# CUHK-AIM-Group/Depth-Aware-Endoscopy-SR

Measured on AMD Instinct MI355X. Metric: LR frames/sec fwd+bwd at x8 (128x160 LR), higher is better.
Workload: dtype f32; 1 GPU; Kvasir x8 synthetic, batch=16 per GPU, fp32, DepthNet nb=16 nf=64 L=256 K=10 (BASELINE.json configs[1]); step = fwd + L1 + dynamic loss + bwd + Adam; global_batch=16, scale=8, parallelism=dp1, mode=train, device=cuda, full=False, hip_graph=False

## Files before the change

### depth-aware-endoscopy-sr_amd/csrc/conv_split_bf16.hip

```cpp
#include "bf16.h"
#include "conv_kernels.h"

typedef _Float16 f16_t;
typedef _Float16 f16x8 __attribute__((ext_vector_type(8)));
typedef _Float16 f16x2_t __attribute__((ext_vector_type(2)));

#define SP_HW 34
#define SP_NWV 8
#define SP_NTHR 512
#define SP_TH 16
#define SP_HPIX (18 * SP_HW)
#define SP_NHP 5
#define SP_HBYTES (SP_NHP * SP_NTHR * 16)
#define SP_EPITCH 144

DASR_DEVICE_CONST __attribute__((aligned(64))) unsigned sp_zero_page[64] = {0};

struct ConvSplitArgs {
    const float* x;
    const bf16_t* ws;
    const float* bias;
    const float* residual;
    float* y;
    int B, H, W, Cin, Cout, accumulate, act, ps_r;
    int tiles_x, tiles_y, nsl, nitems, Q, G8;
    const float* xmax;
    const float* wmax;
    float* ymax;
    const float* xact;
    int fact, fps;
};

template <int N>
__device__ __forceinline__ void sp_wait_vm() {
#ifndef DASR_HIPEMU
    asm volatile("s_waitcnt vmcnt(%0)" ::"n"(N) : "memory");
#endif
}

__device__ __forceinline__ void sp_wait_vm_n(int n) {
    switch (n) {
#define SP_W(N) case N: sp_wait_vm<N>(); break;
        SP_W(0) SP_W(1) SP_W(2) SP_W(3) SP_W(4) SP_W(5) SP_W(6) SP_W(7) SP_W(8) SP_W(9) SP_W(10) SP_W(11) SP_W(12)
#undef SP_W
        default: sp_wait_vm<0>(); break;
    }
}

__device__ __forceinline__ void sp_split3(const float (&x)[8], bf16x8& a0, bf16x8& a1, bf16x8& a2) {
#pragma unroll
    for (int e = 0; e < 8; e += 2) {
        const bf16x2_t h0 = dasr_f2bf2(x[e], x[e + 1]);
        const float r0 = x[e] - dasr_bf2f(h0[0]), r1 = x[e + 1] - dasr_bf2f(h0[1]);
        const bf16x2_t h1 = dasr_f2bf2(r0, r1);
        const float s0 = r0 - dasr_bf2f(h1[0]), s1 = r1 - dasr_bf2f(h1[1]);
        const bf16x2_t h2 = dasr_f2bf2(s0, s1);
        a0[e] = h0[0]; a0[e + 1] = h0[1];
        a1[e] = h1[0]; a1[e + 1] = h1[1];
        a2[e] = h2[0]; a2[e + 1] = h2[1];
    }
}

__host__ __device__ static inline int sp_scale_exp(float m) {
// ... 271 lines not shown
                for (int j = 0; j < 2; ++j) {
                    const int v = lane + 64 * u, cq = v & 7, px = 2 * (v >> 3) + j;
                    const float4 s = *(const float4*)(scr + px * SP_EPITCH + 16 * cq);
                    float o[4] = {s.x, s.y, s.z, s.w};
                    if (NP == 2) {
                        const float* bp = sBias + n0 + 4 * cq;
#pragma unroll
                        for (int t = 0; t < 4; ++t) o[t] = fmaf(o[t], inv, bp[t]);
                    }
                    const float xv[4] = {xa[m][u][j].x, xa[m][u][j].y, xa[m][u][j].z, xa[m][u][j].w};
#pragma unroll
                    for (int t = 0; t < 4; ++t) r[m][u][j][t] = o[t] * (xv[t] > 0.f ? 1.f : dneg);
                }
            DASR_WAVE_SYNC();
        }
        if (rowok) {
            const size_t Cq = (size_t)4 * a.Cout;
#pragma unroll
            for (int u = 0; u < 2; ++u) {
                const int v = lane + 64 * u, cq = v & 7, P = v >> 3;
                if (2 * P >= wvalid) continue;
                float* yp = a.y + (((size_t)bb * (a.H >> 1) + (gy0 >> 1)) * (a.W >> 1) + (x0 >> 1) + P) * Cq + 4 * (n0 + 4 * cq);
#pragma unroll
                for (int t = 0; t < 4; ++t) {
                    const float4 q = make_float4(r[0][u][0][t], r[0][u][1][t], r[1][u][0][t], r[1][u][1][t]);
                    *(float4*)(yp + 4 * t) = q;
                    om = dasr_amax4(om, q);
                }
            }
        }
    }
}

template <int NT, int NP, int RW = 2, int CW = 1>
__global__ void __launch_bounds__(64 * (SP_TH / RW), RW == 4 ? 1 : 2) k_conv3x3_split(ConvSplitArgs a) {
    DASR_DYN_SMEM(smem);
    typedef SpFrag<NP> F;
    static_assert(CW == 1 || (CW == 2 && NP == 2 && RW == 2 && (NT % 2) == 0), "channel halves: fp16 x 2, eight waves");
    constexpr int MR = RW * CW, NW = NT / CW;
    constexpr int NWV = SP_TH / RW, NTHR = 64 * NWV, NHP = SP_HBYTES / (16 * NTHR);
    constexpr int NTILE = 32 * NT, PIECE = NTILE * 32, SLAB = NP * PIECE;
    constexpr int WP = SLAB / 16;
    constexpr int WQ = WP / NTHR, WR = (WP - WQ * NTHR) / 64;
    char* const sH = smem;
    constexpr int TPS = NP == 2 ? 3 : 1, NS = 9 / TPS;
    constexpr int R = 3, D = 2;
    char* const sW = smem + 2 * SP_HBYTES;
    float* const sBias = (float*)(sW + R * TPS * SLAB);
    float* const sRed = sBias + a.Cout;
    const int tid = threadIdx.x, lane = tid & 63, wv = DASR_UNIFORM((int)(tid >> 6));
    const int li = lane & 31, lh = lane >> 5;
    const int wr = wv / CW, wc = wv % CW;
    const int nwq = WQ + (wv < WR ? 1 : 0);
    const dasr_lds_addr_t ldsH = DASR_LDS_ADDR(sH) + 1024 * wv, ldsW = DASR_LDS_ADDR(sW) + 1024 * wv;

    const int xcd = blockIdx.x & 7, jwg = blockIdx.x >> 3;
    const int ibeg = xcd * a.Q;
    const int iend = ibeg + a.Q < a.nitems ? ibeg + a.Q : a.nitems;
    int item = ibeg + jwg;
    if (item >= iend) {
        if (a.ymax) dasr_amax_commit_idle(a.ymax, dasr_flat_wg(), dasr_flat_nwg());
        return;
    }
    const int NC = a.Cin >> 4;
    const int pixb = a.Cin * 4, rowb = a.W * pixb;
    const size_t sampb = (size_t)a.H * rowb;
    const char* const zp = (const char*)sp_zero_page;

    for (int i = tid; i < a.Cout; i += NTHR) sBias[i] = a.bias ? a.bias[i] : 0.f;
    sp_scales_gather<NP>(a.xmax, a.wmax, sRed);
    __syncthreads();
    const SpScale sc = sp_scales_take<NP>(sRed);

    int x0, y0, n0, bb;
    auto decode = [&](int it, int& ox0, int& oy0, int& on0, int& ob) {
        const int ns = it % a.nsl, pt = it / a.nsl;
        const int tile = pt % (a.tiles_x * a.tiles_y);
        ob = pt / (a.tiles_x * a.tiles_y);
        ox0 = (tile % a.tiles_x) * 32;
        oy0 = (tile / a.tiles_x) * SP_TH;
        on0 = ns * NTILE;
    };
    decode(item, x0, y0, n0, bb);
    int hoff[NHP];
    unsigned hok = 0;
    const char* hxb;
    auto halo_setup = [&](int fx0, int fy0, int fb, bool real) {
        hxb = (const char*)a.x + (size_t)fb * sampb;
        const int org = (fy0 - 1) * rowb + (fx0 - 1) * pixb;
        int t = tid;
#ifndef DASR_HIPEMU
        asm volatile("" : "+v"(t));
#endif
        hok = 0;
#pragma unroll
        for (int u = 0; u < NHP; ++u) {
            const int P = (t >> 2) + (NTHR / 4) * u;
            const int pr = P / SP_HW, pc = P - pr * SP_HW;
            hoff[u] = org + pr * rowb + pc * pixb + 16 * ((t & 3) ^ ((P >> 2) & 3));
            const bool ok = real && P < SP_HPIX && (unsigned)(fy0 - 1 + pr) < (unsigned)a.H && (unsigned)(fx0 - 1 + pc) < (unsigned)a.W;
            hok |= ok ? (1u << u) : 0u;
        }
    };
    auto halo_issue = [&](int u, int cc, int buf) {
        const char* src = ((hok >> u) & 1u) ? hxb + hoff[u] + 64 * cc : zp;
// ... 108 lines not shown
                typename F::type A[RW][NP];
#pragma unroll
                for (int m = 0; m < RW; ++m) {
                    const int P = Pq + (m + dy) * SP_HW + dx;
                    const int key = (P >> 2) & 3;
                    if constexpr (NP == 2) {
                        A[m][0] = sp_frag(hb + P * 64, lh, key, 0);
                        A[m][1] = sp_frag(hb + P * 64, lh, key, 1);
                    } else {
                        const float4 lo = *(const float4*)(hb + P * 64 + (((2 * lh) ^ key) << 4));
                        const float4 hi = *(const float4*)(hb + P * 64 + (((2 * lh + 1) ^ key) << 4));
                        const float xv[8] = {lo.x, lo.y, lo.z, lo.w, hi.x, hi.y, hi.z, hi.w};
                        F::split(xv, sc.sx, A[m]);
                    }
                }
                DASR_SETPRIO(1);
#pragma unroll
                for (int n = 0; n < NT; ++n) {
                    typename F::type Bw[NP];
#pragma unroll
                    for (int j = 0; j < NP; ++j) Bw[j] = *(const typename F::type*)(wb + j * PIECE + n * 1024);
#pragma unroll
                    for (int m = 0; m < RW; ++m) acc[m][n] = F::mma(Bw, A[m], acc[m][n]);
                }
                DASR_SETPRIO(0);
                }
                }
            }
            par ^= 1;
        }

        DASR_RAW_BARRIER();
        char* const scr = sH + (par ^ 1) * SP_HBYTES + wv * (32 * SP_EPITCH);
        sp_epilogue<NW, NP, MR>(acc, a, scr, sBias, sc.inv, x0, y0, n0 + 32 * NW * wc, bb, MR * wr, lane, li, lh, om);
        if (!has_next) break;
        item = nitem; x0 = nx0; y0 = ny0; n0 = nn0; bb = nb;
    }
    sp_wait_vm<0>();
    if (a.ymax) dasr_amax_commit(a.ymax, om, sRed, dasr_flat_wg(), dasr_flat_nwg());
}

template <int NP, int NT = 1, bool FUSE = false>
__global__ void __launch_bounds__(SP_NTHR, 2) k_conv3x3_split_n32(ConvSplitArgs a) {
    DASR_DYN_SMEM(smem);
    typedef SpFrag<NP> F;
    constexpr int NTILE = 32 * NT, PIECE = NTILE * 32, SLAB = NP * PIECE;
    constexpr int WCH = 9 * SLAB, WPC = WCH / 16;
    constexpr int WPT = SLAB / 16;
    constexpr int WU = (WPC + SP_NTHR - 1) / SP_NTHR, WLAST = (WPC - (WU - 1) * SP_NTHR) / 64;
    char* const sH = smem;
    char* const sW = smem + 2 * SP_HBYTES;
    float* const sBias = (float*)(sW + 2 * WCH);
    float* const sRed = sBias + a.Cout;
    const int tid = threadIdx.x, lane = tid & 63, wv = DASR_UNIFORM((int)(tid >> 6));
    const int li = lane & 31, lh = lane >> 5;
    const dasr_lds_addr_t ldsH = DASR_LDS_ADDR(sH) + 1024 * wv, ldsW = DASR_LDS_ADDR(sW) + 1024 * wv;

    const int xcd = blockIdx.x & 7, jwg = blockIdx.x >> 3;
    const int ibeg = xcd * a.Q;
    const int iend = ibeg + a.Q < a.nitems ? ibeg + a.Q : a.nitems;
    int item = ibeg + jwg;
    if (item >= iend) {
        if (a.ymax) dasr_amax_commit_idle(a.ymax, dasr_flat_wg(), dasr_flat_nwg());
        return;
    }
    const int NC = a.Cin >> 4;
    const int pixb = a.Cin * 4, rowb = a.W * pixb;
    const size_t sampb = (size_t)a.H * rowb;
    const char* const zp = (const char*)sp_zero_page;

    for (int i = tid; i < a.Cout; i += SP_NTHR) sBias[i] = a.bias ? a.bias[i] : 0.f;
// ... 296 lines not shown
extern "C" int dasr_conv3x3_split2_weights_slabs(int Cin, int Cout) {
    if (Cin <= 0 || Cout <= 0 || (Cin % 32) != 0 || (Cout % 32) != 0) return 0;
    return (int)sp_weight_slabs_all(Cin, Cout);
}
extern "C" int dasr_conv3x3_split2_weights_multi(const dasr_split_job* jobs_host, const dasr_split_job* jobs_device, int njobs,
                                                 void* stream) {
    DASR_CHECK_PTR(jobs_host); DASR_CHECK_PTR(jobs_device);
    DASR_CHECK_SHAPE(njobs > 0);
    long long total = 0;
    for (int j = 0; j < njobs; ++j) {
        const dasr_split_job& J = jobs_host[j];
        DASR_CHECK_PTR(J.w_packed); DASR_CHECK_PTR(J.w_split); DASR_CHECK_PTR(J.wmax);
        DASR_CHECK_SHAPE(J.Cin > 0 && J.Cout > 0 && (J.Cin % 32) == 0 && (J.Cout % 32) == 0);
        DASR_CHECK_SHAPE(J.wg_begin == total);
        total += sp_weight_slabs_all(J.Cin, J.Cout);
        DASR_CHECK_SHAPE(total < (1ll << 30));
    }
    DASR_LAUNCH(k_split_weights_multi, dim3((unsigned)total), dim3(256), 0, stream, jobs_device, njobs);
    DASR_RETURN_LAUNCH_STATUS();
}
template <int NP>
static int sp_launch(ConvSplitArgs& a, void* stream) {
    const int NT = sp_ntile(a.Cout) / 32;
    a.tiles_x = (a.W + 31) / 32;
    a.tiles_y = (a.H + SP_TH - 1) / SP_TH;
    a.nsl = a.Cout / (32 * NT);
    a.nitems = a.tiles_x * a.tiles_y * a.B * a.nsl;
    a.Q = (a.nitems + 7) / 8;
    a.G8 = a.Q < 32 ? a.Q : 32;
    if ((dasr_get_conv_bf16_impl() & 3) == 2) a.G8 = 1;
    const bool chunk2 = NT == 2 && NP == 2 && (dasr_get_conv_bf16_impl() & 512) != 0;
    const size_t lds = 2 * (size_t)SP_HBYTES +
                       (NT == 1 || chunk2 ? 2 * (size_t)(9 * NP * 32 * NT * 32) : 3 * (size_t)((NP == 2 ? 3 : 1) * NP * 32 * NT * 32)) +
                       sizeof(float) * (size_t)(a.Cout + 32);
    if (lds > 160 * 1024) return DASR_E_UNSUPPORTED;
    const dim3 grid(8 * a.G8);
    if (a.xact) {
        if (NT != 1 || NP != 2) return DASR_E_UNSUPPORTED;
        DASR_LAUNCH((k_conv3x3_split_n32<2, 1, true>), grid, dim3(SP_NTHR), lds, stream, a);
    }
    else if (NT == 4 && NP == 2 && (dasr_get_conv_bf16_impl() & 256) != 0)
        DASR_LAUNCH((k_conv3x3_split<4, 2, 4>), grid, dim3(256), lds, stream, a);
    else if (NT == 4 && NP == 2 && (dasr_get_conv_bf16_impl() & 1024) == 0)
        DASR_LAUNCH((k_conv3x3_split<4, 2, 2, 2>), grid, dim3(SP_NTHR), lds, stream, a);
    else if (NT == 2 && NP == 2 && (dasr_get_conv_bf16_impl() & 1024) != 0)
        DASR_LAUNCH((k_conv3x3_split<2, 2, 2, 2>), grid, dim3(SP_NTHR), lds, stream, a);
    else if (NT == 4) DASR_LAUNCH((k_conv3x3_split<4, NP>), grid, dim3(SP_NTHR), lds, stream, a);
    else if (chunk2)  DASR_LAUNCH((k_conv3x3_split_n32<2, 2>), grid, dim3(SP_NTHR), lds, stream, a);
    else if (NT == 2) DASR_LAUNCH((k_conv3x3_split<2, NP>), grid, dim3(SP_NTHR), lds, stream, a);
    else              DASR_LAUNCH((k_conv3x3_split_n32<NP>), grid, dim3(SP_NTHR), lds, stream, a);
    DASR_RETURN_LAUNCH_STATUS();
}
static int sp_fwd(const float* x, const float* xmax, const unsigned short* w_split, const float* wmax, const float* bias,
                  const float* residual, float* y, float* ymax, int B, int H, int W, int Cin, int Cout, int act, int ps_r,
                  void* stream) {
    DASR_CHECK_PTR(x); DASR_CHECK_PTR(w_split); DASR_CHECK_PTR(y);
    DASR_CHECK_SHAPE(B > 0);
    if (!dasr_conv3x3_split_supported(H, W, Cin, Cout)) return DASR_E_UNSUPPORTED;
    if (act < 0 || act > 2) return DASR_E_UNSUPPORTED;
    if (ps_r < 1) ps_r = 1;
    if (ps_r > 2 || (ps_r == 2 && (residual != nullptr || (Cout % 128) != 0))) return DASR_E_UNSUPPORTED;
    ConvSplitArgs a{x, (const bf16_t*)w_split, bias, residual, y, B, H, W, Cin, Cout, 0, act, ps_r, 0, 0, 0, 0, 0, 0, xmax, wmax, ymax};
    return xmax ? sp_launch<2>(a, stream) : sp_launch<3>(a, stream);
}
extern "C" int dasr_conv3x3_fwd_split(const float* x, const unsigned short* w_split, const float* bias,
                                      const float* residual, float* y, int B, int H, int W, int Cin, int Cout, int act,
                                      int ps_r, void* stream) {
    return sp_fwd(x, nullptr, w_split, nullptr, bias, residual, y, nullptr, B, H, W, Cin, Cout, act, ps_r, stream);
}
// ... 9 lines not shown
    DASR_CHECK_SHAPE(B > 0);
    if (!dasr_conv3x3_split_supported(H, W, Cin, Cout)) return DASR_E_UNSUPPORTED;
    const size_t mode1 = (size_t)9 * (dmax ? 2 : 3) * Cin * Cout;
    ConvSplitArgs a{dconv, (const bf16_t*)w_split + mode1, nullptr, nullptr, dx, B, H, W, Cout, Cin,
                    accumulate, DASR_ACT_NONE, 1, 0, 0, 0, 0, 0, 0, dmax, wmax, nullptr};
    return dmax ? sp_launch<2>(a, stream) : sp_launch<3>(a, stream);
}
extern "C" int dasr_conv3x3_dgrad_split(const float* dconv, const unsigned short* w_split, float* dx, int accumulate, int B,
                                        int H, int W, int Cin, int Cout, void* stream) {
    return sp_dgrad(dconv, nullptr, w_split, nullptr, dx, accumulate, B, H, W, Cin, Cout, stream);
}
extern "C" int dasr_conv3x3_dgrad_split2(const float* dconv, const float* dmax, const unsigned short* w_split, const float* wmax,
                                         float* dx, int accumulate, int B, int H, int W, int Cin, int Cout, void* stream) {
    DASR_CHECK_PTR(dmax); DASR_CHECK_PTR(wmax);
    return sp_dgrad(dconv, dmax, w_split, wmax, dx, accumulate, B, H, W, Cin, Cout, stream);
}
extern "C" int dasr_conv3x3_dgrad_act_supported(int H, int W, int Cin, int Cout, int act, int ps_r, int accumulate) {
    if (Cin != 32 || !dasr_conv3x3_split_supported(H, W, Cin, Cout)) return 0;
    if (act != DASR_ACT_NONE && act != DASR_ACT_RELU && act != DASR_ACT_LRELU02) return 0;
    if (ps_r == 1) return 1;
    return (ps_r == 2 && (H % 2) == 0 && (W % 2) == 0 && !accumulate) ? 1 : 0;
}
extern "C" int dasr_conv3x3_dgrad_act_split2(const float* dconv, const float* dmax, const unsigned short* w_split, const float* wmax,
                                             const float* x_act, float* dprev, float* dprev_amax, int accumulate, int B, int H,
                                             int W, int Cin, int Cout, int act, int ps_r, void* stream) {
    DASR_CHECK_PTR(dconv); DASR_CHECK_PTR(dmax); DASR_CHECK_PTR(w_split); DASR_CHECK_PTR(wmax); DASR_CHECK_PTR(x_act);
    DASR_CHECK_PTR(dprev);
    DASR_CHECK_SHAPE(B > 0);
    if (!dasr_conv3x3_dgrad_act_supported(H, W, Cin, Cout, act, ps_r, accumulate)) return DASR_E_UNSUPPORTED;
    const size_t mode1 = (size_t)9 * 2 * Cin * Cout;
    ConvSplitArgs a{dconv, (const bf16_t*)w_split + mode1, nullptr, nullptr, dprev, B, H, W, Cout, Cin,
                    accumulate ? 1 : 0, DASR_ACT_NONE, 1, 0, 0, 0, 0, 0, 0, dmax, wmax, dprev_amax, x_act, act, ps_r};
    return sp_launch<2>(a, stream);
}

#define SW_TW 32
__host__ __device__ constexpr int sw_th(int MT, int NTW) { return MT * NTW == 4 ? 2 : (MT * NTW == 2 ? 4 : 8); }

struct SplitWgradArgs {
    const float* xmax;
    const float* dmax;
    const float* x;
    const float* dy;
    float* slabs;
    float* bslabs;
    int B, H, W, Cin, Cout;
    int P, ntiles;
};

__device__ __forceinline__ void sp_split_pair(float v0, float v1, bf16x2_t& h0, bf16x2_t& h1, bf16x2_t& h2) {
    h0 = dasr_f2bf2(v0, v1);
    const float r0 = v0 - dasr_bf2f(h0[0]), r1 = v1 - dasr_bf2f(h0[1]);
    h1 = dasr_f2bf2(r0, r1);
    h2 = dasr_f2bf2(r0 - dasr_bf2f(h1[0]), r1 - dasr_bf2f(h1[1]));
}

__device__ __forceinline__ void sp_split_pair2(float v0, float v1, float s, f16x2_t& h0, f16x2_t& h1) {
    v0 *= s; v1 *= s;
    h0[0] = (f16_t)v0; h0[1] = (f16_t)v1;
    h1[0] = (f16_t)(v0 - (float)h0[0]); h1[1] = (f16_t)(v1 - (float)h0[1]);
}

template <int MT, int NTW, int NP>
__global__ void __launch_bounds__(256, 2) k_conv3x3_wgrad_split(SplitWgradArgs a) {
    DASR_DYN_SMEM(smem);
    typedef SpFrag<NP> F;
// ... 459 lines not shown
```

### depth-aware-endoscopy-sr_amd/graph.py

```python
import math

import torch

from . import ops
from .tape import Tape, Var, accum


FUSE_DGRAD_ACT = False
FUSE_C9_DGRAD_ACT = True
FUSE_SPLIT_DGRAD_ACT = True

SIDE_STREAM = True
import os as _os
import threading as _threading
TAIL_WGRAD_SIDE = False
FUSE_INSTNORM_STATS = False
ENCODER_S2D = True
SPLIT_BF16 = True
SPLIT_WGRAD = True
SPLIT_PIECES = 2
FUSE_AMAX = True
SPLIT_CONV9 = True
SPLIT_MIN_PIXELS = 1 << 14
WGRAD_STREAM = False
_SIDE = {}
_SIDE_LOCK = _threading.Lock()


def _side_stream(device, which="branch"):
    key = (str(device), which)
    with _SIDE_LOCK:
        if key not in _SIDE:
            _SIDE[key] = torch.cuda.Stream(device=device, priority=-1)
        return _SIDE[key]


def _folded(tape, key, tensors, make):
    cache = tape.fold_cache
    if tape.enabled or cache is None or key is None:
        return make()
    ver = tuple((t.data_ptr(), ops.tensor_version(t)) for t in tensors)
    key = key + (str(tensors[0].device),)
    hit = cache.get(key)
# ... 248 lines not shown
            y = ops.conv3x3_fwd_split(x.data, w.split, bias.data if bias is not None else None, w.data.shape[4],
                                      residual.data if residual is not None else None, act, ps_r)
    elif (SPLIT_BF16 and SPLIT_PIECES == 2 and SPLIT_CONV9 and f32 and w.data.dtype == torch.float32 and stride == 1 and pad == 4
          and not transposed and tuple(w.data.shape[1:3]) == (9, 9) and act == ops.ACT_NONE and ps_r == 1 and residual is None
          and x.data.shape[0] * x.data.shape[1] * x.data.shape[2] >= SPLIT_MIN_PIXELS
          and ops.conv9_split_supported(x.data.shape[1], x.data.shape[2], w.data.shape[3], w.data.shape[4])):
        if w.split is None:
            w.split = ("c9", _folded(tape, ("c9max", "@%x" % w.data.data_ptr()), [w.data], lambda: ops.absmax(w.data[0])))
            if w.pack is not None:
                tape.prepack.note_split(w.pack, w.split)
        y = ops.conv9_fwd_split2(x.data, _amax(x), w.data, w.split[1], bias.data if bias is not None else None)
    else:
        am = want_amax(tape, x.data) if (f32 and x.data.shape[3] in (1, 3) and ps_r == 1) else None
        y = ops.conv2d_fwd(x.data, w.data, bias.data if bias is not None else None,
                           residual.data if residual is not None else None, stride, pad, transposed, act, ps_r, out_dtype,
                           amax=am)
    needs = x.requires_grad or w.requires_grad or (bias is not None and bias.requires_grad) or \
        (residual is not None and residual.requires_grad)
    out = Var(y, needs)
    out.stats = stats
    x.uses += 1
    if residual is not None:
        residual.uses += 1
    if (act != ops.ACT_NONE or ps_r > 1) and residual is None:
        out.epilogue = (act, ps_r)
        out.epilogue_split = isinstance(w.split, tuple)
    if act != ops.ACT_NONE or ps_r > 1:
        out.act_rec = (act, ps_r)
        out.epilogue_split = isinstance(w.split, tuple)
    KH, KW, Cin, Cout = w.data.shape[1:]
    wshape = (KH, KW, Cin, Cout)
    B, H, W_, _ = x.data.shape
    Ho, Wo = ops.conv_out_hw(H, W_, KH, KW, stride, pad, transposed)

    def bwd():
        if out.grad is None:
            return
        dy = out.grad
        out.grad = None
        if out.grad_event is not None:
            torch.cuda.current_stream().wait_event(out.grad_event)
            dy.record_stream(torch.cuda.current_stream())
        if not x.requires_grad and residual is None and ps_r == 1 and act != ops.ACT_NONE:
            dw, db = ops.conv2d_wgrad_act(x.data, dy, y, wshape, act, stride, pad, transposed,
                                          want_bias=bias is not None)
            accum(w, dw)
            if bias is not None:
                accum(bias, db)
            return
        if out.grad_is_preact:
            dconv = dy
        elif act != ops.ACT_NONE or ps_r > 1:
            dconv = ops.conv2d_epilogue_bwd(dy, y, Ho, Wo, Cout, act, ps_r,
                                            amax=want_amax(tape, dy, (B, Ho, Wo, Cout)) if isinstance(w.split, tuple) else None)
        else:
            dconv = dy
        dmax = None
        if w.requires_grad or (bias is not None and bias.requires_grad):
            ws = _side_stream(dconv.device, "wgrad") if (WGRAD_STREAM and dconv.is_cuda) else None
            if ws is None and side_wgrad and TAIL_WGRAD_SIDE and SIDE_STREAM and dconv.is_cuda:
                ws = _side_stream(dconv.device)
            if ws is None and _is_c9(w):
                dmax = _amax_t(dconv)
                dw, db = ops.conv9_wgrad_split2(x.data, _amax(x), dconv, dmax, want_bias=bias is not None)
            elif ws is None and w.split is not None and SPLIT_WGRAD:
                if isinstance(w.split, tuple):
                    dmax = _amax_t(dconv)
                    dw, db = ops.conv3x3_wgrad_split2(x.data, _amax(x), dconv, dmax, want_bias=bias is not None)
                else:
                    dw, db = ops.conv3x3_wgrad_split(x.data, dconv, want_bias=bias is not None)
            elif ws is None:
                dw, db = ops.conv2d_wgrad(x.data, dconv, wshape, stride, pad, transposed, want_bias=bias is not None)
            else:
                cur = torch.cuda.current_stream()
                ready = cur.record_event()
                if ws not in tape.side_streams:
                    tape.side_streams.append(ws)
                with torch.cuda.stream(ws):
                    ws.wait_event(ready)
                    dconv.record_stream(ws)
                    dw, db = ops.conv2d_wgrad(x.data, dconv, wshape, stride, pad, transposed,
                                              want_bias=bias is not None)
                    done = ws.record_event()
                w.grad_event = done
                if bias is not None:
                    bias.grad_event = done
            accum(w, dw)
            if bias is not None:
                accum(bias, db)
        if x.requires_grad:
            if (FUSE_DGRAD_ACT and f32 and x.grad is None and x.uses == 1 and x.epilogue is not None and
                    ops.conv2d_dgrad_act_supported(x.data.shape, w.data, dconv.shape, stride, pad, transposed,
                                                   x.epilogue[1])):
                x.grad = ops.conv2d_dgrad_act(dconv, w.data, x.data, x.epilogue[0], x.epilogue[1], stride, pad,
                                              transposed)
                x.grad_is_preact = True
            elif (_is_c9(w) and FUSE_C9_DGRAD_ACT and x.grad is None and x.uses == 1 and x.epilogue is not None
                  and ops.conv9_dgrad_act_supported(x.data.shape, Cout, x.epilogue[0], x.epilogue[1])):
                if dmax is None:
                    dmax = _amax_t(dconv)
                x.grad = ops.conv9_dgrad_act_split2(dconv, dmax, w.data, w.split[1], x.data, x.epilogue[0], x.epilogue[1],
                                                    amax=want_amax(tape, dconv, (B, H // 2, W_ // 2, 4 * Cin))
                                                    if x.epilogue_split else None)
                x.grad_is_preact = True
            elif (FUSE_SPLIT_DGRAD_ACT and isinstance(w.split, tuple) and not _is_c9(w) and Cin == 32 and f32
                  and x.act_rec is not None and x.grads_in + 1 == x.uses
                  and ops.conv3x3_dgrad_act_supported(x.data.shape, Cout, x.act_rec[0], x.act_rec[1], x.grad is not None)):
                if dmax is None:
                    dmax = _amax_t(dconv)
                r = x.act_rec[1]
                x.grad = ops.conv3x3_dgrad_act_split2(dconv, dmax, w.split, x.data, x.act_rec[0], r, out=x.grad,
                                                      amax=want_amax(tape, dconv, (B, H // r, W_ // r, r * r * Cin))
                                                      if x.epilogue_split else None)
                x.grad_is_preact = True
            elif _is_c9(w):
                if dmax is None:
                    dmax = _amax_t(dconv)
                x.grad = ops.conv9_dgrad_split2(dconv, dmax, w.data, w.split[1], x.data.shape, out=x.grad)
            elif isinstance(w.split, tuple):
                if dmax is None:
                    dmax = _amax_t(dconv)
                x.grad = ops.conv3x3_dgrad_split2(dconv, dmax, w.split, x.data.shape, out=x.grad)
            elif w.split is not None:
                if x.grad is None:
# ... 460 lines not shown
```

### depth-aware-endoscopy-sr_amd/ops.py

```python
import ctypes

import torch

from . import _lib

ACT_NONE, ACT_RELU, ACT_LRELU = 0, 1, 2
IN_EPS = 1e-5


BF16 = torch.bfloat16


def _p(t, allow_none=False):
    return _lib.ptr(t, allow_none)


def _pa(t, allow_none=False):
    if t is None:
        return _lib.ptr(t, allow_none)
    return _lib.ptr(t, allow_none, dtype=t.dtype if t.dtype in (torch.float32, BF16) else torch.float32)


def _is_bf(*ts):
    kinds = {t.dtype for t in ts if t is not None}
# ... 494 lines not shown
    _call("dasr_conv3x3_wgrad_split2", _p(x), _p(xmax), _p(dconv), _p(dmax), _p(dw), _p(db, True), _p(ws), nbytes, B, H, W, Cin,
          Cout)
    return dw, db


def conv3x3_dgrad_split2(dconv, dmax, ws, x_shape, out=None):
    B, H, W, Cin = x_shape
    Cout = dconv.shape[3]
    acc = out is not None
    if out is None:
        out = empty(tuple(x_shape), dconv)
    drop_amax(out)
    _call("dasr_conv3x3_dgrad_split2", _p(dconv), _p(dmax), _lib.ptr(ws[0], False, torch.float16), _p(ws[1]), _p(out), 1 if acc else 0, B, H, W, Cin, Cout)
    return out


def conv3x3_dgrad_act_supported(x_shape, Cout, act, ps_r, accumulate=False):
    B, H, W, Cin = x_shape
    return bool(_lib.get().dasr_conv3x3_dgrad_act_supported(H, W, Cin, Cout, act, ps_r, 1 if accumulate else 0))


def conv3x3_dgrad_act_split2(dconv, dmax, ws, x_act, act, ps_r, out=None, amax=None):
    B, H, W, Cin = x_act.shape
    Cout = dconv.shape[3]
    acc = out is not None
    if out is None:
        out = empty((B, H // 2, W // 2, 4 * Cin) if ps_r == 2 else (B, H, W, Cin), dconv)
    drop_amax(out)
    _call("dasr_conv3x3_dgrad_act_split2", _p(dconv), _p(dmax), _lib.ptr(ws[0], False, torch.float16), _p(ws[1]), _p(x_act),
          _p(out), _p(amax, True), 1 if acc else 0, B, H, W, Cin, Cout, act, ps_r)
    return set_amax(out, amax)


def conv9_split_supported(H, W, Cin, Cout):
    return bool(_lib.get().dasr_conv9_split_supported(H, W, Cin, Cout))


def conv9_fwd_split2(x, xmax, w, wmax, bias):
    B, H, W, Cin = x.shape
    Cout = w.shape[4]
    y = empty((B, H, W, Cout), x)
    _call("dasr_conv9_fwd_split2", _p(x), _p(xmax), _p(w), _p(wmax), _p(bias, True), _p(y), B, H, W, Cin, Cout)
    return y


def conv9_dgrad_split2(dconv, dmax, w, wmax, x_shape, out=None):
    B, H, W, Cin = x_shape
    Cout = dconv.shape[3]
    acc = out is not None
    if out is None:
        out = empty(tuple(x_shape), dconv)
    drop_amax(out)
    _call("dasr_conv9_dgrad_split2", _p(dconv), _p(dmax), _p(w), _p(wmax), _p(out), 1 if acc else 0, B, H, W, Cin, Cout)
    return out


def conv9_dgrad_act_supported(x_shape, Cout, act, ps_r):
    B, H, W, Cin = x_shape
    return (ps_r == 2 and H % 2 == 0 and W % 2 == 0 and act in (ACT_NONE, ACT_RELU, ACT_LRELU)
            and conv9_split_supported(H, W, Cin, Cout))


def conv9_dgrad_act_split2(dconv, dmax, w, wmax, x_act, act, ps_r, amax=None):
    B, H, W, Cin = x_act.shape
    Cout = dconv.shape[3]
    dprev = empty((B, H // 2, W // 2, 4 * Cin), dconv)
# ... 326 lines not shown
```

### depth-aware-endoscopy-sr_amd/tape.py

```python
from . import ops


class Var:
    __slots__ = ("data", "grad", "requires_grad", "name", "uses", "epilogue", "grad_is_preact", "event",
                 "grad_event", "stats", "split", "amax", "pack", "epilogue_split", "act_rec", "grads_in")

    def __init__(self, data, requires_grad=False, name=None):
        self.data = data
        self.grad = None
        self.requires_grad = requires_grad
        self.name = name
        self.uses = 0
        self.epilogue = None
        self.epilogue_split = False
        self.act_rec = None
        self.grads_in = 0
        self.grad_is_preact = False
        self.event = None
        self.grad_event = None
        self.stats = None
        self.split = None
        self.amax = None
        self.pack = None

    @property
    def shape(self):
        return self.data.shape


class Tape:

    def __init__(self, enabled=True, act_dtype=None):
        import torch
        self.enabled = enabled
        self.act_dtype = act_dtype if act_dtype is not None else torch.float32
        self.nodes = []
        self._stream = None
        self.side_streams = []
        self.fold_cache = None
        self.prepack = None
        self.marks = []
        self.on_mark = None

    def record(self, fn):
        if self.enabled:
            self.nodes.append((fn, self._stream))

    def mark(self):
# ... 51 lines not shown
```

### include/dasr.h

```cpp
#ifndef DASR_H
#define DASR_H

#include <stddef.h>
#include <stdint.h>

#ifdef __cplusplus
extern "C" {
#endif

#define DASR_OK 0
#define DASR_E_NULL (-1)
#define DASR_E_SHAPE (-2)
#define DASR_E_UNSUPPORTED (-3)
#define DASR_E_WORKSPACE (-4)

#define DASR_ACT_NONE 0
#define DASR_ACT_RELU 1
#define DASR_ACT_LRELU02 2

int dasr_version(void);
const char* dasr_error_string(int code);
int dasr_is_device_build(void);

int dasr_nchw_to_nhwc(const float* src, float* dst, int B, int C, int H, int W, void* stream);
// ... 50 lines not shown
int dasr_conv3x3_split_weights(const float* w_packed, unsigned short* w_split, int Cin, int Cout, void* stream);
int dasr_conv3x3_fwd_split(const float* x, const unsigned short* w_split, const float* bias, const float* residual, float* y,
                           int B, int H, int W, int Cin, int Cout, int act, int ps_r, void* stream);
int dasr_conv3x3_dgrad_split(const float* dconv, const unsigned short* w_split, float* dx, int accumulate, int B, int H,
                             int W, int Cin, int Cout, void* stream);
size_t dasr_conv3x3_wgrad_split_workspace(int B, int H, int W, int Cin, int Cout);
int dasr_conv3x3_wgrad_split(const float* x, const float* dconv, float* dw_hwio, float* dbias, void* workspace,
                             size_t workspace_bytes, int B, int H, int W, int Cin, int Cout, void* stream);

#define DASR_AMAX_MAX_PARTS 4096
#define DASR_AMAX_FLOATS (1 + DASR_AMAX_MAX_PARTS)
int dasr_absmax(const float* x, size_t n, float* amax, void* stream);
size_t dasr_conv3x3_split2_weights_bytes(int Cin, int Cout);
int dasr_conv3x3_split2_weights(const float* w_packed, const float* wmax, unsigned short* w_split, int Cin, int Cout,
                                void* stream);
typedef struct dasr_split_job {
    const float* w_packed; const float* wmax; unsigned short* w_split;
    int Cin, Cout, wg_begin, reserved;
} dasr_split_job;
int dasr_conv3x3_split2_weights_slabs(int Cin, int Cout);
int dasr_conv3x3_split2_weights_multi(const dasr_split_job* jobs_host, const dasr_split_job* jobs_device, int njobs, void* stream);
int dasr_conv3x3_fwd_split2(const float* x, const float* xmax, const unsigned short* w_split, const float* wmax,
                            const float* bias, const float* residual, float* y, float* y_amax, int B, int H, int W, int Cin,
                            int Cout, int act, int ps_r, void* stream);
int dasr_conv3x3_dgrad_split2(const float* dconv, const float* dmax, const unsigned short* w_split, const float* wmax,
                              float* dx, int accumulate, int B, int H, int W, int Cin, int Cout, void* stream);
int dasr_conv3x3_wgrad_split2(const float* x, const float* xmax, const float* dconv, const float* dmax, float* dw_hwio,
                              float* dbias, void* workspace, size_t workspace_bytes, int B, int H, int W, int Cin, int Cout,
                              void* stream);
int dasr_conv3x3_dgrad_act_supported(int H, int W, int Cin, int Cout, int act, int ps_r, int accumulate);
int dasr_conv3x3_dgrad_act_split2(const float* dconv, const float* dmax, const unsigned short* w_split, const float* wmax,
                                  const float* x_act, float* dprev, float* dprev_amax, int accumulate, int B, int H, int W,
                                  int Cin, int Cout, int act, int ps_r, void* stream);

int dasr_conv9_split_supported(int H, int W, int Cin, int Cout);
int dasr_conv9_fwd_split2(const float* x, const float* xmax, const float* w_hwio, const float* wmax, const float* bias, float* y,
                          int B, int H, int W, int Cin, int Cout, void* stream);
int dasr_conv9_dgrad_split2(const float* dconv, const float* dmax, const float* w_hwio, const float* wmax, float* dx,
                            int accumulate, int B, int H, int W, int Cin, int Cout, void* stream);
int dasr_conv9_dgrad_act_split2(const float* dconv, const float* dmax, const float* w_hwio, const float* wmax, const float* x_act,
                                float* dprev, float* amax, int B, int H, int W, int Cin, int Cout, int act, int ps_r,
                                void* stream);
size_t dasr_conv9_wgrad_split2_workspace(int B, int H, int W, int Cin, int Cout);
int dasr_conv9_wgrad_split2(const float* x, const float* xmax, const float* dconv, const float* dmax, float* dw_hwio, float* dbias,
                            void* workspace, size_t workspace_bytes, int B, int H, int W, int Cin, int Cout, void* stream);

size_t dasr_instnorm_stats_workspace(int B, int HW, int C);
int dasr_instnorm_stats(const float* x, float* mean, float* var, void* workspace, size_t workspace_bytes, int B, int HW,
                        int C, void* stream);

int dasr_dynk_fwd(const float* st, const float* A_w, const float* A_b, const float* W_gamma, const float* W_beta,
                  float* stp, float* D, int B, int K, int L, int C, void* stream);
int dasr_dynk_bwd(const float* dD, const float* st, const float* stp, const float* A_w, const float* W_gamma,
                  const float* W_beta, float* dW_gamma, float* dW_beta, float* dA_w, float* dA_b, float* dst,
                  float* dstp, int B, int K, int L, int C, void* stream);

int dasr_mask_compress(const float* mask, unsigned char* region, int* onehot_flag, int B, int K, int H, int W,
                       void* stream);
int dasr_sean_fwd(const float* t, const float* mean, const float* var, const float* gb2, const float* mask,
                  const unsigned char* region, const int* onehot_flag, const float* D, const float* bias_gamma, const float* bias_beta, const float* alpha_gamma,
                  const float* alpha_beta, const float* residual, float* out, float* out_amax, int relu, int B, int H,
                  int W, int C, int K, float eps, void* stream);
size_t dasr_sean_bwd_workspace(int B, int H, int W, int C, int K);
int dasr_sean_bwd(const float* dout, const float* out, const float* t, const float* mean, const float* var,
                  const float* gb2, const float* mask, const unsigned char* region, const int* onehot_flag,
                  const float* D, const float* bias_gamma, const float* bias_beta,
// ... 107 lines not shown
```

Before: 262.9 frames/s.

## Fuse depth-mask conv weight gradient into the following conv's dgrad epilogue

The input-gradient kernel of a 3x3 conv whose input comes from a 1-channel depth conv (Cin=128) now also computes that producer conv's weight and bias gradients in its epilogue. The epilogue applies the activation derivative, then accumulates depth-patch times gradient products with fp32 MFMA, writing per-workgroup partial slabs that a small reduce kernel sums. This removes the materialised producer gradient tensor and the separate wgrad_act pass over it. In exchange the epilogue carries extra LDS, registers and global reads of depth and activations.

Result: no change. 265.3 frames/s (median of 6 runs) (+0.9%).

```diff
diff --git a/depth-aware-endoscopy-sr_amd/csrc/conv_split_bf16.hip b/depth-aware-endoscopy-sr_amd/csrc/conv_split_bf16.hip
--- a/depth-aware-endoscopy-sr_amd/csrc/conv_split_bf16.hip
+++ b/depth-aware-endoscopy-sr_amd/csrc/conv_split_bf16.hip
@@ -29,6 +29,8 @@
     float* ymax;
     const float* xact;
     int fact, fps;
+    const float* depth;
+    float* c1w;
 };
 
 template <int N>
@@ -366,11 +368,91 @@
     }
 }
 
-template <int NT, int NP, int RW = 2, int CW = 1>
+#define SP_C1W_HALO ((4 + 2) * SP_HW)
+template <int NW, int MR>
+__device__ __forceinline__ void sp_epilogue_c1w(f32x16 (&acc)[MR][NW], f32x4 (&dacc)[2 * NW], const ConvSplitArgs& a, char* const scr,
+                                                const float* sOZ, float* sD, const float inv, const int x0, const int y0,
+                                                const int nb, const int bb, const int rbase, const int lane, const int li,
+                                                const int lh) {
+    static_assert(MR == 4, "four tile rows per wave");
+    const int wvalid = a.W - x0;
+    const float dneg = a.fact == DASR_ACT_RELU ? 0.f : (a.fact == DASR_ACT_LRELU02 ? 0.2f : 1.f);
+    const float4 z4 = make_float4(0.f, 0.f, 0.f, 0.f);
+    float dv[4];
+#pragma unroll
+    for (int q = 0; q < 4; ++q) {
+        const int i = lane + 64 * q, r = i / SP_HW, c = i - r * SP_HW;
+        const int gy = y0 - 1 + rbase + r, gx = x0 - 1 + c;
+        dv[q] = 0.f;
+        if (i < SP_C1W_HALO && (unsigned)gy < (unsigned)a.H && (unsigned)gx < (unsigned)a.W)
+            dv[q] = a.depth[((size_t)bb * a.H + gy) * a.W + gx];
+    }
+    DASR_WAVE_SYNC();
+#pragma unroll
+    for (int q = 0; q < 4; ++q)
+        if (lane + 64 * q < SP_C1W_HALO) sD[lane + 64 * q] = dv[q];
+    const int t = lane & 15, kq = lane >> 4;
+    const float* const ap = t < 9 ? sD + (t / 3) * SP_HW + (t % 3) + kq : sOZ + (t == 9 ? 0 : 32) + kq;
+    const int astr = t < 9 ? SP_HW : 0;
+    DASR_WAVE_SYNC();
+#pragma unroll
+    for (int m = 0; m < MR; ++m) {
+        const int gy = y0 + rbase + m;
+        float Af[8];
+#pragma unroll
+        for (int j = 0; j < 8; ++j) Af[j] = ap[m * astr + 4 * j];
+#pragma unroll
+        for (int n = 0; n < NW; ++n) {
+            float4 xa[2][2];
+            bool ok[2];
+#pragma unroll
+            for (int u = 0; u < 2; ++u) {
+                const int v = lane + 64 * u, pix = v >> 2, cg = v & 3;
+                ok[u] = gy < a.H && pix < wvalid;
+                const size_t idx = (((size_t)bb * a.H + gy) * a.W + x0 + pix) * a.Cout + nb + 32 * n + 8 * cg;
+                xa[u][0] = z4; xa[u][1] = z4;
+                if (ok[u]) { xa[u][0] = *(const float4*)(a.xact + idx); xa[u][1] = *(const float4*)(a.xact + idx + 4); }
+            }
+#pragma unroll
+            for (int g = 0; g < 4; ++g) {
+                f32x4 pk = {acc[m][n][4 * g], acc[m][n][4 * g + 1], acc[m][n][4 * g + 2], acc[m][n][4 * g + 3]};
+                *(f32x4*)(scr + li * SP_EPITCH + (8 * g + 4 * lh) * 4) = pk;
+            }
+            DASR_WAVE_SYNC();
+#pragma unroll
+            for (int u = 0; u < 2; ++u) {
+                const int v = lane + 64 * u, pix = v >> 2, cg = v & 3;
+                float4* const sp = (float4*)(scr + pix * SP_EPITCH + 32 * cg);
+                const float4 lo = sp[0], hi = sp[1];
+                float o[8] = {lo.x, lo.y, lo.z, lo.w, hi.x, hi.y, hi.z, hi.w};
+                const float xv[8] = {xa[u][0].x, xa[u][0].y, xa[u][0].z, xa[u][0].w, xa[u][1].x, xa[u][1].y, xa[u][1].z, xa[u][1].w};
+#pragma unroll
+                for (int e = 0; e < 8; ++e) {
+                    const float gq = (o[e] * inv) * (xv[e] > 0.f ? 1.f : dneg);
+                    o[e] = ok[u] ? gq : 0.f;
+                }
+                sp[0] = make_float4(o[0], o[1], o[2], o[3]);
+                sp[1] = make_float4(o[4], o[5], o[6], o[7]);
+            }
+            DASR_WAVE_SYNC();
+#pragma unroll
+            for (int j = 0; j < 8; ++j)
+#pragma unroll
+                for (int cb = 0; cb < 2; ++cb) {
+                    const float bq = *(const float*)(scr + (4 * j + kq) * SP_EPITCH + (16 * cb + t) * 4);
+                    dacc[2 * n + cb] = __builtin_amdgcn_mfma_f32_16x16x4f32(Af[j], bq, dacc[2 * n + cb], 0, 0, 0);
+                }
+            DASR_WAVE_SYNC();
+        }
+    }
+}
+
+template <int NT, int NP, int RW = 2, int CW = 1, bool C1W = false>
 __global__ void __launch_bounds__(64 * (SP_TH / RW), RW == 4 ? 1 : 2) k_conv3x3_split(ConvSplitArgs a) {
     DASR_DYN_SMEM(smem);
     typedef SpFrag<NP> F;
     static_assert(CW == 1 || (CW == 2 && NP == 2 && RW == 2 && (NT % 2) == 0), "channel halves: fp16 x 2, eight waves");
+    static_assert(!C1W || (CW == 2 && NT == 4), "the fused weight gradient: 128 produced channels, channel halves");
     constexpr int MR = RW * CW, NW = NT / CW;
     constexpr int NWV = SP_TH / RW, NTHR = 64 * NWV, NHP = SP_HBYTES / (16 * NTHR);
     constexpr int NTILE = 32 * NT, PIECE = NTILE * 32, SLAB = NP * PIECE;
@@ -382,6 +464,7 @@
     char* const sW = smem + 2 * SP_HBYTES;
     float* const sBias = (float*)(sW + R * TPS * SLAB);
     float* const sRed = sBias + a.Cout;
+    float* const sC1 = sRed + 32;
     const int tid = threadIdx.x, lane = tid & 63, wv = DASR_UNIFORM((int)(tid >> 6));
     const int li = lane & 31, lh = lane >> 5;
     const int wr = wv / CW, wc = wv % CW;
@@ -394,6 +477,8 @@
     int item = ibeg + jwg;
     if (item >= iend) {
         if (a.ymax) dasr_amax_commit_idle(a.ymax, dasr_flat_wg(), dasr_flat_nwg());
+        if constexpr (C1W)
+            for (int i = tid; i < 10 * 128; i += NTHR) a.c1w[(size_t)blockIdx.x * (10 * 128) + i] = 0.f;
         return;
     }
     const int NC = a.Cin >> 4;
@@ -403,8 +488,12 @@
 
     for (int i = tid; i < a.Cout; i += NTHR) sBias[i] = a.bias ? a.bias[i] : 0.f;
     sp_scales_gather<NP>(a.xmax, a.wmax, sRed);
+    if (C1W && tid < 64) sC1[tid] = tid < 32 ? 1.f : 0.f;
     __syncthreads();
     const SpScale sc = sp_scales_take<NP>(sRed);
+    f32x4 dacc[NT];
+#pragma unroll
+    for (int i = 0; i < NT; ++i) dacc[i] = f32x4{0.f, 0.f, 0.f, 0.f};
 
     int x0, y0, n0, bb;
     auto decode = [&](int it, int& ox0, int& oy0, int& on0, int& ob) {
@@ -579,11 +668,27 @@
 
         DASR_RAW_BARRIER();
         char* const scr = sH + (par ^ 1) * SP_HBYTES + wv * (32 * SP_EPITCH);
-        sp_epilogue<NW, NP, MR>(acc, a, scr, sBias, sc.inv, x0, y0, n0 + 32 * NW * wc, bb, MR * wr, lane, li, lh, om);
+        if constexpr (C1W)
+            sp_epilogue_c1w<NW, MR>(acc, dacc, a, scr, sC1, sC1 + 64 + wv * SP_C1W_HALO, sc.inv, x0, y0, n0 + 32 * NW * wc, bb,
+                                    MR * wr, lane, li, lh);
+        else
+            sp_epilogue<NW, NP, MR>(acc, a, scr, sBias, sc.inv, x0, y0, n0 + 32 * NW * wc, bb, MR * wr, lane, li, lh, om);
         if (!has_next) break;
         item = nitem; x0 = nx0; y0 = ny0; n0 = nn0; bb = nb;
     }
     sp_wait_vm<0>();
+    if constexpr (C1W) {
+        DASR_LDS_BARRIER();
+        float* const red = (float*)sW;
+#pragma unroll
+        for (int i = 0; i < NT; ++i)
+#pragma unroll
+            for (int r = 0; r < 4; ++r)
+                red[(wr * 16 + (lane >> 4) * 4 + r) * 128 + 32 * NW * wc + 16 * i + (lane & 15)] = dacc[i][r];
+        DASR_LDS_BARRIER();
+        for (int i = tid; i < 10 * 128; i += NTHR)
+            a.c1w[(size_t)blockIdx.x * (10 * 128) + i] = ((red[i] + red[2048 + i]) + red[4096 + i]) + red[6144 + i];
+    }
     if (a.ymax) dasr_amax_commit(a.ymax, om, sRed, dasr_flat_wg(), dasr_flat_nwg());
 }
 
@@ -946,9 +1051,14 @@
     const bool chunk2 = NT == 2 && NP == 2 && (dasr_get_conv_bf16_impl() & 512) != 0;
     const size_t lds = 2 * (size_t)SP_HBYTES +
                        (NT == 1 || chunk2 ? 2 * (size_t)(9 * NP * 32 * NT * 32) : 3 * (size_t)((NP == 2 ? 3 : 1) * NP * 32 * NT * 32)) +
-                       sizeof(float) * (size_t)(a.Cout + 32);
+                       sizeof(float) * (size_t)(a.Cout + 32) + (a.c1w ? sizeof(float) * (size_t)(64 + SP_NWV * SP_C1W_HALO) : 0);
     if (lds > 160 * 1024) return DASR_E_UNSUPPORTED;
     const dim3 grid(8 * a.G8);
+    if (a.c1w) {
+        if (NT != 4 || NP != 2 || a.nsl != 1) return DASR_E_UNSUPPORTED;
+        DASR_LAUNCH((k_conv3x3_split<4, 2, 2, 2, true>), grid, dim3(SP_NTHR), lds, stream, a);
+        DASR_RETURN_LAUNCH_STATUS();
+    }
     if (a.xact) {
         if (NT != 1 || NP != 2) return DASR_E_UNSUPPORTED;
         DASR_LAUNCH((k_conv3x3_split_n32<2, 1, true>), grid, dim3(SP_NTHR), lds, stream, a);
@@ -1024,6 +1134,47 @@
     ConvSplitArgs a{dconv, (const bf16_t*)w_split + mode1, nullptr, nullptr, dprev, B, H, W, Cout, Cin,
                     accumulate ? 1 : 0, DASR_ACT_NONE, 1, 0, 0, 0, 0, 0, 0, dmax, wmax, dprev_amax, x_act, act, ps_r};
     return sp_launch<2>(a, stream);
+}
+__global__ void __launch_bounds__(256) k_c1w_reduce(const float* __restrict__ slabs, int nslab, float* __restrict__ dw,
+                                                    float* __restrict__ dbias) {
+    DASR_DYN_SMEM(smem);
+    float* const part = (float*)smem;
+    const int l = threadIdx.x & 63, sg = threadIdx.x >> 6, o = blockIdx.x * 64 + l;
+    float s = 0.f;
+#pragma unroll 8
+    for (int k = sg; k < nslab; k += 4) s += slabs[(size_t)k * (10 * 128) + o];
+    part[sg * 64 + l] = s;
+    __syncthreads();
+    if (sg == 0) {
+        const float r = ((part[l] + part[64 + l]) + part[128 + l]) + part[192 + l];
+        if (o < 9 * 128) dw[o] = r;
+        else if (dbias) dbias[o - 9 * 128] = r;
+    }
+}
+extern "C" int dasr_conv3x3_dgrad_c1wgrad_supported(int H, int W, int Cin, int Cout, int act, int depth_channels) {
+    if (Cin != 128 || depth_channels != 1 || Cout <= 0 || !dasr_conv3x3_split_supported(H, W, Cin, Cout)) return 0;
+    return (act == DASR_ACT_NONE || act == DASR_ACT_RELU || act == DASR_ACT_LRELU02) ? 1 : 0;
+}
+extern "C" size_t dasr_conv3x3_dgrad_c1wgrad_workspace(int B, int H, int W) {
+    if (B <= 0 || H <= 0 || W <= 0) return 0;
+    return sizeof(float) * (size_t)(10 * 128) * 8 * 32;
+}
+extern "C" int dasr_conv3x3_dgrad_c1wgrad_split2(const float* dconv, const float* dmax, const unsigned short* w_split,
+                                                 const float* wmax, const float* x_act, const float* depth, float* dw_mask,
+                                                 float* dbias_mask, void* workspace, int B, int H, int W, int Cin, int Cout,
+                                                 int act, void* stream) {
+    DASR_CHECK_PTR(dconv); DASR_CHECK_PTR(dmax); DASR_CHECK_PTR(w_split); DASR_CHECK_PTR(wmax); DASR_CHECK_PTR(x_act);
+    DASR_CHECK_PTR(depth); DASR_CHECK_PTR(dw_mask); DASR_CHECK_PTR(workspace);
+    DASR_CHECK_SHAPE(B > 0);
+    if (!dasr_conv3x3_dgrad_c1wgrad_supported(H, W, Cin, Cout, act, 1)) return DASR_E_UNSUPPORTED;
+    const size_t mode1 = (size_t)9 * 2 * Cin * Cout;
+    ConvSplitArgs a{dconv, (const bf16_t*)w_split + mode1, nullptr, nullptr, nullptr, B, H, W, Cout, Cin,
+                    0, DASR_ACT_NONE, 1, 0, 0, 0, 0, 0, 0, dmax, wmax, nullptr, x_act, act, 1, depth, (float*)workspace};
+    const int rc = sp_launch<2>(a, stream);
+    if (rc != 0) return rc;
+    DASR_LAUNCH(k_c1w_reduce, dim3(10 * 128 / 64), dim3(256), sizeof(float) * 256, stream, (const float*)workspace,
+                8 * a.G8, dw_mask, dbias_mask);
+    DASR_RETURN_LAUNCH_STATUS();
 }
 
 #define SW_TW 32
diff --git a/depth-aware-endoscopy-sr_amd/graph.py b/depth-aware-endoscopy-sr_amd/graph.py
--- a/depth-aware-endoscopy-sr_amd/graph.py
+++ b/depth-aware-endoscopy-sr_amd/graph.py
@@ -9,6 +9,7 @@
 FUSE_DGRAD_ACT = False
 FUSE_C9_DGRAD_ACT = True
 FUSE_SPLIT_DGRAD_ACT = True
+FUSE_MASK_WGRAD = True
 
 SIDE_STREAM = True
 import os as _os
@@ -323,6 +324,10 @@
     wshape = (KH, KW, Cin, Cout)
     B, H, W_, _ = x.data.shape
     Ho, Wo = ops.conv_out_hw(H, W_, KH, KW, stride, pad, transposed)
+    leaf = not x.requires_grad and residual is None and ps_r == 1 and act != ops.ACT_NONE
+    if (leaf and needs and f32 and Cin == 1 and (KH, KW) == (3, 3) and stride == 1 and pad == 1 and not transposed
+            and x.data.dtype == torch.float32):
+        out.producer = (x.data, w, bias, act)
 
     def bwd():
         if out.grad is None:
@@ -332,7 +337,7 @@
         if out.grad_event is not None:
             torch.cuda.current_stream().wait_event(out.grad_event)
             dy.record_stream(torch.cuda.current_stream())
-        if not x.requires_grad and residual is None and ps_r == 1 and act != ops.ACT_NONE:
+        if leaf:
             dw, db = ops.conv2d_wgrad_act(x.data, dy, y, wshape, act, stride, pad, transposed,
                                           want_bias=bias is not None)
             accum(w, dw)
@@ -380,7 +385,17 @@
             if bias is not None:
                 accum(bias, db)
         if x.requires_grad:
-            if (FUSE_DGRAD_ACT and f32 and x.grad is None and x.uses == 1 and x.epilogue is not None and
+            if (FUSE_MASK_WGRAD and isinstance(w.split, tuple) and not _is_c9(w) and f32 and x.producer is not None
+                    and x.uses == 1 and x.grad is None
+                    and ops.conv3x3_dgrad_c1wgrad_supported(x.data.shape, Cout, x.producer[3], x.producer[0].shape[3])):
+                if dmax is None:
+                    dmax = _amax_t(dconv)
+                p_depth, p_w, p_bias, p_act = x.producer
+                dwm, dbm = ops.conv3x3_dgrad_c1wgrad_split2(dconv, dmax, w.split, x.data, p_depth, p_act,
+                                                            want_bias=p_bias is not None and p_bias.requires_grad)
+                accum(p_w, dwm)
+                accum(p_bias, dbm)
+            elif (FUSE_DGRAD_ACT and f32 and x.grad is None and x.uses == 1 and x.epilogue is not None and
                     ops.conv2d_dgrad_act_supported(x.data.shape, w.data, dconv.shape, stride, pad, transposed,
                                                    x.epilogue[1])):
                 x.grad = ops.conv2d_dgrad_act(dconv, w.data, x.data, x.epilogue[0], x.epilogue[1], stride, pad,
diff --git a/depth-aware-endoscopy-sr_amd/ops.py b/depth-aware-endoscopy-sr_amd/ops.py
--- a/depth-aware-endoscopy-sr_amd/ops.py
+++ b/depth-aware-endoscopy-sr_amd/ops.py
@@ -550,6 +550,29 @@
     return set_amax(out, amax)
 
 
+def conv3x3_dgrad_c1wgrad_supported(x_shape, Cout, act, depth_channels=1):
+    B, H, W, Cin = x_shape
+    return bool(_lib.get().dasr_conv3x3_dgrad_c1wgrad_supported(H, W, Cin, Cout, act, depth_channels))
+
+
+def conv3x3_dgrad_c1wgrad_workspace(B, H, W):
+    return int(_lib.get().dasr_conv3x3_dgrad_c1wgrad_workspace(B, H, W))
+
+
+def conv3x3_dgrad_c1wgrad_split2(dconv, dmax, ws, x_act, depth, act, want_bias=True):
+    B, H, W, Cin = x_act.shape
+    Cout = dconv.shape[3]
+    if tuple(depth.shape[:3]) != (B, H, W) or not conv3x3_dgrad_c1wgrad_supported(x_act.shape, Cout, act, depth.shape[3]):
+        raise RuntimeError("dasr_conv3x3_dgrad_c1wgrad_split2: unsupported shapes %s, %s, %s, act %d" %
+                           (tuple(x_act.shape), tuple(depth.shape), tuple(dconv.shape), act))
+    wk = torch.empty((conv3x3_dgrad_c1wgrad_workspace(B, H, W) // 4,), dtype=torch.float32, device=dconv.device)
+    dw = empty((3, 3, 1, Cin), dconv)
+    db = empty((Cin,), dconv) if want_bias else None
+    _call("dasr_conv3x3_dgrad_c1wgrad_split2", _p(dconv), _p(dmax), _lib.ptr(ws[0], False, torch.float16), _p(ws[1]), _p(x_act),
+          _p(depth), _p(dw), _p(db, True), _p(wk), B, H, W, Cin, Cout, act)
+    return dw, db
+
+
 def conv9_split_supported(H, W, Cin, Cout):
     return bool(_lib.get().dasr_conv9_split_supported(H, W, Cin, Cout))
 
diff --git a/depth-aware-endoscopy-sr_amd/tape.py b/depth-aware-endoscopy-sr_amd/tape.py
--- a/depth-aware-endoscopy-sr_amd/tape.py
+++ b/depth-aware-endoscopy-sr_amd/tape.py
@@ -3,7 +3,7 @@
 
 class Var:
     __slots__ = ("data", "grad", "requires_grad", "name", "uses", "epilogue", "grad_is_preact", "event",
-                 "grad_event", "stats", "split", "amax", "pack", "epilogue_split", "act_rec", "grads_in")
+                 "grad_event", "stats", "split", "amax", "pack", "epilogue_split", "act_rec", "grads_in", "producer")
 
     def __init__(self, data, requires_grad=False, name=None):
         self.data = data
@@ -14,6 +14,7 @@
         self.epilogue = None
         self.epilogue_split = False
         self.act_rec = None
+        self.producer = None
         self.grads_in = 0
         self.grad_is_preact = False
         self.event = None
diff --git a/include/dasr.h b/include/dasr.h
--- a/include/dasr.h
+++ b/include/dasr.h
@@ -106,6 +106,11 @@
 int dasr_conv3x3_dgrad_act_split2(const float* dconv, const float* dmax, const unsigned short* w_split, const float* wmax,
                                   const float* x_act, float* dprev, float* dprev_amax, int accumulate, int B, int H, int W,
                                   int Cin, int Cout, int act, int ps_r, void* stream);
+int dasr_conv3x3_dgrad_c1wgrad_supported(int H, int W, int Cin, int Cout, int act, int depth_channels);
+size_t dasr_conv3x3_dgrad_c1wgrad_workspace(int B, int H, int W);
+int dasr_conv3x3_dgrad_c1wgrad_split2(const float* dconv, const float* dmax, const unsigned short* w_split, const float* wmax,
+                                      const float* x_act, const float* depth, float* dw_mask, float* dbias_mask, void* workspace,
+                                      int B, int H, int W, int Cin, int Cout, int act, void* stream);
 
 int dasr_conv9_split_supported(int H, int W, int Cin, int Cout);
 int dasr_conv9_fwd_split2(const float* x, const float* xmax, const float* w_hwio, const float* wmax, const float* bias, float* y,
```
